# chagmgang/distributed_reinforcement_learning

Hardware: AMD Instinct MI355X
Metric: learner env-frames/sec (whole node), IMPALA deep-conv 84x84x4 (higher is better)
Workload: dtype bf16; 1 GPU; model=impala deep-conv 84x84x4 + LSTM256 V-trace, global_batch=32, seq_len=20, parallelism=dp1, num_action=18

## Files before the change

distributed_reinforcement_learning_amd/ops/conv_op.py:

```python

from __future__ import annotations

import torch

from distributed_reinforcement_learning_amd import ops as _ops

_LAYER_CO = {0: 32, 1: 32, 2: 64, 3: 64}

_WGRAD_STREAM = None


def _side_enabled() -> bool:
    import os
    return os.environ.get("DRLA_WGRAD_SIDE") == "1"


def wgrad_stream() -> torch.cuda.Stream:
    global _WGRAD_STREAM
    if _WGRAD_STREAM is None:
        _WGRAD_STREAM = torch.cuda.Stream()
    return _WGRAD_STREAM


def join_wgrad_stream() -> None:
    if _WGRAD_STREAM is not None:
        torch.cuda.current_stream().wait_stream(_WGRAD_STREAM)


STASH_INPUTS = False


class _ConvLayer(torch.autograd.Function):
    @staticmethod
    def forward(ctx, x: torch.Tensor, w_flat: torch.Tensor,
                bias_f32: torch.Tensor, layer: int):
        ext = _ops.require_ext()
        stash = STASH_INPUTS and layer <= 1
        y, x_st = ext.conv_fwd(layer, x.contiguous(), w_flat.contiguous(),
                               bias_f32.contiguous(), stash)
        ctx.save_for_backward(x_st if stash else x, w_flat, y)
        ctx.layer = layer
        return y

    @staticmethod
    def backward(ctx, dy: torch.Tensor):
        x, w_flat, y = ctx.saved_tensors
        ext = _ops.require_ext()
        layer = ctx.layer
        co = _LAYER_CO[layer]
        if not (dy.is_contiguous() or (dy.stride(-1) == 1
                                        and dy.dim() >= 2)):
            dy = dy.contiguous()
        dy_m = ext.relu_mask_bwd(dy, y, co, layer)
        if _side_enabled():
            cur = torch.cuda.current_stream()
            side = wgrad_stream()
            side.wait_stream(cur)
            with torch.cuda.stream(side):
                dw, dbias = ext.conv_wgrad(layer, x, dy_m)
            if not torch.cuda.is_current_stream_capturing():
                cur.wait_stream(side)
                for t in (dw, dbias):
                    t.record_stream(cur)
                for t in (x, dy_m):
                    t.record_stream(side)
        else:
            dw, dbias = ext.conv_wgrad(layer, x, dy_m)
        dx = None
        if layer >= 2 and ctx.needs_input_grad[0]:
            dx = ext.conv_dgrad(layer, dy_m, w_flat)
        return dx, dw, dbias, None


def conv_layer(x: torch.Tensor, conv: torch.nn.Conv2d,
               layer: int) -> torch.Tensor:
    w = conv.weight
    co = w.shape[0]
    w_flat = w.permute(0, 2, 3, 1).reshape(co, -1)
    return _ConvLayer.apply(x, w_flat, conv.bias, layer)


def atari_conv_stack(stack, x_u8_nhwc: torch.Tensor) -> torch.Tensor:
    ci = x_u8_nhwc.shape[-1]
    l1 = 0 if ci == 4 else 1
    y = conv_layer(x_u8_nhwc, stack.conv1, l1)
    y = conv_layer(y, stack.conv2, 2)
    y = conv_layer(y, stack.conv3, 3)
    return y.reshape(y.shape[0], -1)


def custom_stack_ok(stack, x: torch.Tensor) -> bool:
    return (x.is_cuda and x.dtype == torch.uint8
            and x.shape[1] == 84 and x.shape[2] == 84
            and x.shape[3] in (1, 4)
            and stack.conv1.weight.dtype == torch.bfloat16
            and _ops.available())
```

distributed_reinforcement_learning_amd/ops/hip/bind.cpp:

```cpp

#include <torch/extension.h>
#include <ATen/hip/HIPContext.h>
#include <hip/hip_runtime.h>

#include <algorithm>
#include <array>
#include <tuple>

#include "drla_kernels.h"

namespace {

hipStream_t cur_stream() {
  return at::hip::getCurrentHIPStream().stream();
}

void check_gpu_contig(const torch::Tensor& t, const char* name) {
  TORCH_CHECK(t.is_cuda(), name, " must be on the GPU");
  TORCH_CHECK(t.is_contiguous(), name, " must be contiguous");
}

template <typename... Ts>
void check_all_gpu_contig(const char* what, const Ts&... ts) {
  (check_gpu_contig(ts, what), ...);
// ... 133 lines not shown
                       0, cur_stream(), BF16P(in), BF16P(w), BF16P(bias),
                       BF16PM(out), batch);
  }
  return {out, x_stash};
}

static torch::Tensor& dbias_slot_buf(const torch::Tensor& like,
                                     int64_t slot_id) {
  static torch::Tensor bufs[4];
  TORCH_CHECK(slot_id >= 0 && slot_id < 4, "bad slot id");
  if (!bufs[slot_id].defined()) {
    bufs[slot_id] =
        torch::zeros({DRLA_DBIAS_SLOTS * DRLA_DBIAS_STRIDE},
                     like.options().dtype(torch::kFloat));
  }
  return bufs[slot_id];
}

torch::Tensor relu_mask_bwd(torch::Tensor dy, torch::Tensor y, int64_t CO,
                            int64_t slot_id) {
  check_gpu_contig(y, "y");
  TORCH_CHECK(dy.is_cuda(), "dy must be on GPU");
  long long n_stride, row_elems;
  if (dy.is_contiguous()) {
    n_stride = row_elems = dy.numel() / dy.size(0);
  } else {
    row_elems = 1;
    for (int d = 1; d < dy.dim(); ++d) {
      TORCH_CHECK(dy.stride(d - 1) >= dy.stride(d), "dy must be row-major");
      row_elems *= dy.size(d);
    }
    TORCH_CHECK(dy.stride(dy.dim() - 1) == 1 &&
                    dy.stride(0) >= row_elems && row_elems % 8 == 0,
                "dy view must be inner-contiguous");
    for (int d = 1; d + 1 < dy.dim(); ++d) {
      TORCH_CHECK(dy.stride(d) == dy.size(d + 1) * dy.stride(d + 1),
                  "dy inner dims must be contiguous");
    }
    n_stride = dy.stride(0);
  }
  auto out = torch::empty(dy.sizes(), dy.options());
  auto& slots = dbias_slot_buf(dy, slot_id);
  const long long n = dy.numel();
  TORCH_CHECK(n % 8 == 0, "relu_mask_bwd wants numel % 8 == 0");
  int grid = drla_grid(n / 8);
  if (grid > 640) grid = 640;
  hipLaunchKernelGGL(drla_relu_mask_bwd, dim3(grid), dim3(DRLA_BLOCK),
                     0, cur_stream(), BF16P(dy), BF16P(y), BF16PM(out),
                     slots.data_ptr<float>(), n, (int)CO, n_stride,
                     row_elems);
  return out;
}

std::tuple<torch::Tensor, torch::Tensor> conv_wgrad(int layer,
                                                    torch::Tensor in,
                                                    torch::Tensor dy) {
  check_gpu_contig(in, "in");
  check_gpu_contig(dy, "dy");
  const auto& cfg = conv_layer(layer);
  const int batch = in.size(0);
  const int K = cfg.kh * cfg.kw * cfg.ci;
  static int split_env = [] {
    const char* e = getenv("DRLA_WGRAD_SPLIT");
    return e ? atoi(e) : 0;
  }();
  const int split = split_env ? split_env : ((layer <= 1) ? 512 : 64);
  static torch::Tensor scratch_cache[4];
  if (!scratch_cache[layer].defined()) {
    scratch_cache[layer] =
        torch::zeros({K, cfg.co}, dy.options().dtype(torch::kFloat));
  }
  auto scratch = scratch_cache[layer];
  const dim3 grid((K + DRLA_CONV_WGRAD_BK - 1) / DRLA_CONV_WGRAD_BK, split);
  if (layer <= 1) {
    hipLaunchKernelGGL(kConvWgradU8[layer], grid, dim3(DRLA_CONV_BLOCK), 0,
                       cur_stream(), in.data_ptr<uint8_t>(), BF16P(dy),
                       scratch.data_ptr<float>(), batch);
  } else {
    hipLaunchKernelGGL(kConvWgradBf16[layer - 2], grid,
                       dim3(DRLA_CONV_BLOCK), 0, cur_stream(), BF16P(in),
                       BF16P(dy), scratch.data_ptr<float>(), batch);
  }
  auto dw = torch::empty({cfg.co, K}, dy.options().dtype(torch::kBFloat16));
  auto dbias = torch::empty({cfg.co}, dy.options().dtype(torch::kBFloat16));
  auto& slots = dbias_slot_buf(dy, layer);
  hipLaunchKernelGGL(drla_wgrad_finalize,
                     dim3(drla_grid((long long)K * cfg.co)),
                     dim3(DRLA_BLOCK), 0, cur_stream(),
                     scratch.data_ptr<float>(), BF16PM(dw), K, cfg.co,
                     slots.data_ptr<float>(), BF16PM(dbias));
  return {dw, dbias};
}

torch::Tensor conv_dgrad(int layer, torch::Tensor dy, torch::Tensor w) {
  check_gpu_contig(dy, "dy");
  check_gpu_contig(w, "w");
  TORCH_CHECK(layer == 2 || layer == 3, "dgrad only for l2/l3");
  const auto& cfg = conv_layer(layer);
  const int batch = dy.size(0);
  auto dx = torch::empty({batch, cfg.hi, cfg.wi, cfg.ci},
                         dy.options().dtype(torch::kBFloat16));
  if (layer == 2) {
    const int grid_c = conv_m_tiles(batch * (cfg.hi / 2) * (cfg.wi / 2));
    hipLaunchKernelGGL(drla_conv_dgrad_l2, dim3(grid_c, 4),
                       dim3(DRLA_CONV_BLOCK), 0, cur_stream(), BF16P(dy),
                       BF16P(w), BF16PM(dx), batch);
  } else {
    hipLaunchKernelGGL(drla_conv_dgrad_l3,
                       dim3(conv_m_tiles(batch * cfg.hi * cfg.wi)),
                       dim3(DRLA_CONV_BLOCK), 0, cur_stream(), BF16P(dy),
                       BF16P(w), BF16PM(dx), batch);
  }
  return dx;
}

std::tuple<torch::Tensor, torch::Tensor> dqn_loss_fwd(
    torch::Tensor main_q, torch::Tensor next_main, torch::Tensor next_tgt,
    torch::Tensor actions, torch::Tensor rewards, torch::Tensor discounts,
    torch::Tensor weights) {
  check_all_gpu_contig("dqn_loss input", main_q, next_main, next_tgt,
                       actions, rewards, discounts, weights);
  TORCH_CHECK(actions.scalar_type() == torch::kInt, "actions must be i32");
  const int B = main_q.size(0), A = main_q.size(1);
  const DualPtr mq = dual_ptr(main_q);
  auto fopt = rewards.options().dtype(torch::kFloat);
  auto loss = torch::zeros({1}, fopt);
  auto td = torch::empty({B}, fopt);
  hipLaunchKernelGGL(
      drla_dqn_loss_fwd, dim3((B + 255) / 256), dim3(256), 0, cur_stream(),
      mq.bf16, mq.f32, next_main.data_ptr<float>(), next_tgt.data_ptr<float>(),
      actions.data_ptr<int>(), rewards.data_ptr<float>(),
      discounts.data_ptr<float>(), weights.data_ptr<float>(),
      loss.data_ptr<float>(), td.data_ptr<float>(), B, A);
  return {loss, td};
}

torch::Tensor dqn_loss_bwd(torch::Tensor td, torch::Tensor actions,
                           torch::Tensor weights, torch::Tensor gloss,
                           int64_t A, bool want_bf16) {
  check_all_gpu_contig("dqn_loss bwd input", td, actions, weights, gloss);
  const int B = td.numel();
  auto dmq = torch::empty(
      {B, A},
      td.options().dtype(want_bf16 ? torch::kBFloat16 : torch::kFloat));
  const DualPtr out = dual_ptr(dmq);
  hipLaunchKernelGGL(
      drla_dqn_loss_bwd, dim3(((long long)B * A + 255) / 256), dim3(256), 0,
      cur_stream(), td.data_ptr<float>(), actions.data_ptr<int>(),
      weights.data_ptr<float>(), gloss.data_ptr<float>(), out.bf16, out.f32,
      B, (int)A);
  return dmq;
}

std::tuple<torch::Tensor, torch::Tensor, torch::Tensor> a2c_loss_fwd(
    torch::Tensor logits, torch::Tensor value, torch::Tensor next_value,
    torch::Tensor actions, torch::Tensor rewards, torch::Tensor done,
    double gamma, int64_t clip_mode, double c_bl, double c_ent) {
  check_all_gpu_contig("a2c loss input", logits, value, next_value, actions,
                       rewards, done);
  TORCH_CHECK(actions.scalar_type() == torch::kInt, "actions must be i32");
  TORCH_CHECK(done.scalar_type() == torch::kBool, "done must be bool");
  const int N = logits.size(0), A = logits.size(1);
  const DualPtr lg = dual_ptr(logits);
  auto fopt = value.options().dtype(torch::kFloat);
// ... 757 lines not shown
                     norm_buf.data_ptr<float>(), static_cast<float>(clip),
                     lr_buf.data_ptr<float>(), static_cast<float>(rho),
                     static_cast<float>(eps), n);
}

void rmsprop_step(torch::Tensor p, torch::Tensor g, torch::Tensor ms,
                  double clip, double lr, double rho, double eps) {
  auto lr_buf = torch::full({1}, lr, p.options());
  rmsprop_step_t(p, g, ms, clip, lr_buf, rho, eps);
}

void adam_step_t(torch::Tensor p, torch::Tensor g, torch::Tensor m,
                 torch::Tensor v, double clip, torch::Tensor lr_buf,
                 double beta1, double beta2, double eps) {
  check_all_gpu_contig("adam tensor", p, g, m, v, lr_buf);
  const long long n = p.numel();
  torch::Tensor norm_buf;
  if (clip > 0) {
    norm_buf = sq_norm(g);
  } else {
    norm_buf = torch::zeros({1}, p.options());
  }
  hipLaunchKernelGGL(drla_adam_step, dim3(drla_grid(n)), dim3(DRLA_BLOCK), 0,
                     cur_stream(), p.data_ptr<float>(), g.data_ptr<float>(),
                     m.data_ptr<float>(), v.data_ptr<float>(),
                     norm_buf.data_ptr<float>(), static_cast<float>(clip),
                     lr_buf.data_ptr<float>(), static_cast<float>(beta1),
                     static_cast<float>(beta2), static_cast<float>(eps), n);
}

void adam_step(torch::Tensor p, torch::Tensor g, torch::Tensor m,
               torch::Tensor v, double clip, double lr_t, double beta1,
               double beta2, double eps) {
  auto lr_buf = torch::full({1}, lr_t, p.options());
  adam_step_t(p, g, m, v, clip, lr_buf, beta1, beta2, eps);
}

}

PYBIND11_MODULE(TORCH_EXTENSION_NAME, m) {
  m.def("normalize_frames_f32", &normalize_frames_f32,
        "uint8 frames -> float32/255 (K11)");
  m.def("normalize_frames_bf16", &normalize_frames_bf16,
        "uint8 frames -> bf16/255 (K11)");
  m.def("vtrace_scan", &vtrace_scan, "fused V-trace reverse scan (K5)");
  m.def("vtrace_loss_fwd", &vtrace_loss_fwd,
        "fused IMPALA loss pipeline forward (K5+K7+K13)");
  m.def("vtrace_loss_bwd", &vtrace_loss_bwd,
        "fused IMPALA loss pipeline backward (closed form)");
  m.def("mfma_probe", &mfma_probe, "16x16x32 bf16 MFMA layout probe");
  m.def("conv_fwd", &conv_fwd,
        "MFMA implicit-GEMM conv fwd, fused normalize+bias+ReLU (K1)");
  m.def("conv_wgrad", &conv_wgrad, "MFMA conv weight gradient (K1 bwd)");
  m.def("conv_dgrad", &conv_dgrad, "MFMA conv data gradient (K1 bwd)");
  m.def("relu_mask_bwd", &relu_mask_bwd,
        "fused-ReLU backward mask + bias gradient");
  m.def("dqn_loss_fwd", &dqn_loss_fwd,
        "fused double-DQN target + IS-weighted TD loss (K8)");
  m.def("dqn_loss_bwd", &dqn_loss_bwd, "closed-form K8 backward");
  m.def("a2c_loss_fwd", &a2c_loss_fwd, "fused A2C loss fwd (K6)");
  m.def("a2c_loss_bwd", &a2c_loss_bwd, "fused A2C loss bwd (K6)");
  m.def("r2d2_loss_fwd", &r2d2_loss_fwd,
        "fused R2D2 sequence-TD tail fwd (K9; n_step > 1 or "
        "priority_eta >= 0 selects the n-step kernel)",
        py::arg("mq"), py::arg("tq"), py::arg("actions"), py::arg("rewards"),
        py::arg("done"), py::arg("weights"), py::arg("gamma"),
        py::arg("clip_mode"), py::arg("n_step") = 1,
        py::arg("priority_eta") = -1.0);
  m.def("dhead_train_fwd", &dhead_train_fwd,
        "grad-carrying dueling head fwd (R2D2 trained window)");
  m.def("dhead_train_bwd", &dhead_train_bwd,
        "grad-carrying dueling head bwd chain + weight grads");
  m.def("dueling_head_fwd", &dueling_head_fwd,
        "no-grad dueling head over the post-burn-in window");
  m.def("r2d2_loss_bwd", &r2d2_loss_bwd,
        "fused R2D2 sequence-TD tail bwd (K9)");
  m.def("per_update", &per_update, "GPU PER segment-tree batched update");
  m.def("per_sample", &per_sample, "GPU PER stratified sample descent");
  m.def("multi_gather", &multi_gather,
        "one-kernel replay batch gather (all fields)");
  m.def("per_rebuild", &per_rebuild,
        "GPU PER interior-sum rebuild (float32 drift repair)");
  m.def("embed_bwd", &embed_bwd,
        "action-embedding table gradient (K2 backward)");
  m.def("lstm_tail_fwd", &lstm_tail_fwd, "fused LSTM gate tail fwd (K3)");
  m.def("lstm_tail_bwd", &lstm_tail_bwd, "fused LSTM gate tail bwd (K3)");
  m.def("mlp_heads_fwd", &mlp_heads_fwd,
        "fused policy+value MLP heads forward (K4)");
  m.def("mlp_heads_bwd", &mlp_heads_bwd,
        "fused heads dgrad chain + ReLU masks + bias grads (K4 bwd)");
  m.def("embed_mlp_fwd", &embed_mlp_fwd,
        "fused action-embedding MLP forward (K2)");
  m.def("embed_mlp_bwd", &embed_mlp_bwd,
        "fused action-embedding MLP backward (K2 bwd)");
  m.def("mlp_heads_pack_wt", &mlp_heads_pack_wt,
        "one-kernel transposed-weight pack for the heads dgrad");
  m.def("mlp_heads_wgrad", &mlp_heads_wgrad,
        "all six head wgrads (dW = dz^T @ act) in one MFMA launch");
  m.def("lstm_seq_train_fwd", &lstm_seq_train_fwd,
        "grad-carrying whole-sequence LSTM forward (K3 seq, R2D2 train)");
  m.def("lstm_seq_train_bwd", &lstm_seq_train_bwd,
        "whole-sequence LSTM backward (one kernel over the recurrence)");
  m.def("lstm_seq_fwd", &lstm_seq_fwd,
        "whole no-grad LSTM unroll in one kernel (K3 seq / burn-in)");
  m.def("sq_norm", &sq_norm, "squared L2 norm of a flat tensor (K12)");
  m.def("grad_gather", &grad_gather,
        "one-kernel scattered-grad -> flat bucket pack (K12b)");
// ... 15 lines not shown
```

distributed_reinforcement_learning_amd/ops/hip/conv.hip:

```cpp

#include "drla_kernels.h"

#define CONV_KERNEL \
  extern "C" __global__ __launch_bounds__(DRLA_CONV_BLOCK) void

__device__ __forceinline__ float cv_bf2f(bf16raw u) {
  unsigned int x = ((unsigned int)u) << 16;
  return __uint_as_float(x);
}

extern "C" __global__ void drla_mfma_probe(const bf16raw* __restrict__ A,
                                           const bf16raw* __restrict__ B,
                                           float* __restrict__ D) {
  const int l = threadIdx.x;
  bf16x8 a_frag, b_frag;
  for (int e = 0; e < 8; ++e) {
    a_frag[e] = (short)A[(l & 15) * 32 + ((l >> 4) * 8 + e)];
    b_frag[e] = (short)B[((l >> 4) * 8 + e) * 16 + (l & 15)];
  }
  f32x4 acc = {0.f, 0.f, 0.f, 0.f};
  acc = __builtin_amdgcn_mfma_f32_16x16x32_bf16(a_frag, b_frag, acc, 0, 0, 0);
  for (int r = 0; r < 4; ++r) {
    D[((l >> 4) * 4 + r) * 16 + (l & 15)] = acc[r];
  }
// ... 242 lines not shown
    long long si = i;
    if (strided) {
      const long long r = i / row8;
      si = (r * n_stride + (i - r * row8) * 8) / 8;
    }
    const uint4 dv = dy4[si];
    const uint4 yv = y4[i];
    uint4 ov;
    DRLA_RM_LANE(dv.x, yv.x, ov.x, acc[0], acc[1]);
    DRLA_RM_LANE(dv.y, yv.y, ov.y, acc[2], acc[3]);
    DRLA_RM_LANE(dv.z, yv.z, ov.z, acc[4], acc[5]);
    DRLA_RM_LANE(dv.w, yv.w, ov.w, acc[6], acc[7]);
    out4[i] = ov;
  }
#undef DRLA_RM_LANE
  __shared__ float red[DRLA_BLOCK * 8];
  for (int e = 0; e < 8; ++e) red[tid * 8 + e] = acc[e];
  __syncthreads();
  if (tid < CO) {
    const int g = tid / 8;
    const int e = tid % 8;
    float s = 0.0f;
    for (int t = g; t < DRLA_BLOCK; t += CO / 8) s += red[t * 8 + e];
    atomicAdd(&dbias_slots[(blockIdx.x & (DRLA_DBIAS_SLOTS - 1)) *
                               DRLA_DBIAS_STRIDE +
                           tid], s);
  }
}

extern "C" __global__ void drla_wgrad_finalize(
    float* __restrict__ scratch, bf16raw* __restrict__ dw, int K,
    int CO, float* __restrict__ dbias_slots,
    bf16raw* __restrict__ dbias) {
  if (dbias_slots && blockIdx.x == 0 && (int)threadIdx.x < CO) {
    float s = 0.0f;
    for (int t = 0; t < DRLA_DBIAS_SLOTS; ++t) {
      s += dbias_slots[t * DRLA_DBIAS_STRIDE + threadIdx.x];
      dbias_slots[t * DRLA_DBIAS_STRIDE + threadIdx.x] = 0.0f;
    }
    dbias[threadIdx.x] = drla_f32_to_bf16(s);
  }
  long long i = blockIdx.x * (long long)blockDim.x + threadIdx.x;
  const long long total = (long long)K * CO;
  const long long stride = gridDim.x * (long long)blockDim.x;
  for (; i < total; i += stride) {
    const int co = i / K;
    const int k = i - (long long)co * K;
    const long long si = (long long)k * CO + co;
    dw[i] = drla_f32_to_bf16(scratch[si]);
    scratch[si] = 0.0f;
  }
}


template <typename IN_T, int CI, int CO, int KH, int KW, int STRIDE, int HI,
          int WI, int HO, int WO>
__device__ void conv_wgrad_impl(const IN_T* __restrict__ in,
                                const bf16raw* __restrict__ dy,
                                float* __restrict__ scratch,
                                int batch) {
  constexpr int K = KH * KW * CI;
  constexpr int BKM = 64;
  constexpr int BKK = DRLA_CONV_WGRAD_BK;
  constexpr int PAD = 8;
  constexpr int NFRAG = CO / 16;
  constexpr int CO_PER_T = (CO * 32) / DRLA_CONV_BLOCK;
  const int M = batch * HO * WO;

  __shared__ bf16raw Am[2][BKK][BKM + PAD];
  __shared__ bf16raw BmT[2][CO][BKM + PAD];

  const int tid = threadIdx.x;
  const int wave = tid / 64;
  const int lane = tid % 64;
  const int k_row0 = blockIdx.x * BKK;

  f32x4 acc[NFRAG];
  for (int ni = 0; ni < NFRAG; ++ni) acc[ni] = {0.f, 0.f, 0.f, 0.f};

  const int m_per_split = (M + gridDim.y - 1) / gridDim.y;
  const int m_begin = blockIdx.y * m_per_split;
  const int m_end = min(M, m_begin + m_per_split);

  const int a_m = tid >> 2;
  const int a_k = (tid & 3) * 16;
  long long a_off0 = 0, a_off1 = 0;
  long long a_offc[16];
  if constexpr (CI == 4) {
    const int kb = k_row0 + a_k;
    const int kh = kb / (KW * CI);
    a_off0 = (long long)kh * WI + (kb - kh * KW * CI) / CI;
  } else if constexpr (CI == 1) {
    static_assert(K % BKK == 0,
                  "CI==1 contiguous row staging requires K % BKK == 0");
#pragma unroll
    for (int t = 0; t < 16; ++t) {
      const int k2 = k_row0 + a_k + t;
      const int kh = k2 / KW;
      a_offc[t] = (k2 < K) ? (long long)kh * WI + (k2 - kh * KW) : -1;
    }
  } else {
    const int kk0 = k_row0 + a_k;
    const int kh0 = kk0 / (KW * CI);
    const int kwci0 = kk0 - kh0 * KW * CI;
    a_off0 = (kk0 < K)
        ? ((long long)kh0 * WI + kwci0 / CI) * CI + (kwci0 % CI) : -1;
// ... 144 lines not shown
  load_chunk(m_begin);
  store_chunk(0);
  load_chunk(m_begin + BKM);
  __syncthreads();
  int nchunks = 0;
  for (int m0 = m_begin; m0 < m_end; m0 += BKM) ++nchunks;
  for (int t = 0; t < nchunks; ++t) {
    const int cur = t & 1;
    if (t + 1 < nchunks) {
      store_chunk(1 - cur);
      load_chunk(m_begin + (long long)(t + 2) * BKM);
    }
    for (int kk = 0; kk < BKM; kk += 32) {
      const bf16x8 a_frag = *reinterpret_cast<const bf16x8*>(
          &Am[cur][wave * 16 + (lane & 15)][kk + (lane >> 4) * 8]);
      for (int ni = 0; ni < NFRAG; ++ni) {
        const int co = ni * 16 + (lane & 15);
        const bf16x8 b_frag = *reinterpret_cast<const bf16x8*>(
            &BmT[cur][co][kk + (lane >> 4) * 8]);
        acc[ni] = __builtin_amdgcn_mfma_f32_16x16x32_bf16(a_frag, b_frag,
                                                          acc[ni], 0, 0, 0);
      }
    }
    __syncthreads();
  }

  for (int ni = 0; ni < NFRAG; ++ni) {
    const int co = ni * 16 + (lane & 15);
    for (int r = 0; r < 4; ++r) {
      const int k = k_row0 + wave * 16 + (lane >> 4) * 4 + r;
      if (k < K) atomicAdd(&scratch[(long long)k * CO + co], acc[ni][r]);
    }
  }
}

CONV_KERNEL drla_conv_wgrad_l1(
    const unsigned char* in, const bf16raw* dy, float* scratch, int batch) {
  conv_wgrad_impl<unsigned char, DRLA_CONV_GEOM(0)>(in, dy, scratch, batch);
}
CONV_KERNEL drla_conv_wgrad_l1_c1(
    const unsigned char* in, const bf16raw* dy, float* scratch, int batch) {
  conv_wgrad_impl<unsigned char, DRLA_CONV_GEOM(1)>(in, dy, scratch, batch);
}
CONV_KERNEL drla_conv_wgrad_l2(
    const bf16raw* in, const bf16raw* dy, float* scratch, int batch) {
  conv_wgrad_impl<bf16raw, DRLA_CONV_GEOM(2)>(in, dy, scratch, batch);
}
CONV_KERNEL drla_conv_wgrad_l3(
    const bf16raw* in, const bf16raw* dy, float* scratch, int batch) {
  conv_wgrad_impl<bf16raw, DRLA_CONV_GEOM(3)>(in, dy, scratch, batch);
}


template <int CI, int CO, int KH, int KW, int STRIDE, int HI, int WI, int HO,
          int WO>
__device__ void conv_dgrad_impl(const bf16raw* __restrict__ dy,
                                const bf16raw* __restrict__ w,
                                bf16raw* __restrict__ dx,
                                int batch) {
  constexpr int K = KH * KW * CI;
  constexpr int Kg = KH * KW * CO;
  constexpr int BM = DRLA_CONV_BM;
  constexpr int BK = 32;
  constexpr int PAD = 8;
  constexpr int NFRAG = CI / 16;
  const int M2 = batch * HI * WI;

  __shared__ bf16raw Ad[BM][BK + PAD];
  __shared__ bf16raw Bd[CI][BK + PAD];

  const int tid = threadIdx.x;
  const int wave = tid / 64;
  const int lane = tid % 64;
  const int row0 = blockIdx.x * BM;

  f32x4 acc[2][NFRAG];
  for (int mi = 0; mi < 2; ++mi)
    for (int ni = 0; ni < NFRAG; ++ni)
      acc[mi][ni] = {0.f, 0.f, 0.f, 0.f};

  const int a_row = tid >> 1;
  const int a_k0 = (tid & 1) * 16;
  const int m2 = row0 + a_row;
  const int n_idx = m2 / (HI * WI);
  const int rem = m2 - n_idx * (HI * WI);
  const int hi = rem / WI;
  const int wi = rem - hi * WI;

  uint4 rda0, rda1;
  bf16raw rbw[8];
  constexpr int CI_PER_T = (CI * BK) / DRLA_CONV_BLOCK;
  const int b_col = tid % BK;
  const int b_ci0 = (tid / BK) * CI_PER_T;

  auto load_chunk = [&](int kg0) {
    const int tap = kg0 / CO;
    const int co0 = kg0 - tap * CO;
    const int kh = tap / KW;
    const int kw = tap - kh * KW;
    bool valid = (m2 < M2);
    int ho = 0, wo = 0;
    if (valid) {
      const int hh = hi - kh;
      const int ww = wi - kw;
      valid = hh >= 0 && ww >= 0 && (hh % STRIDE) == 0 && (ww % STRIDE) == 0;
      if (valid) {
        ho = hh / STRIDE;
        wo = ww / STRIDE;
        valid = ho < HO && wo < WO;
      }
    }
    if (valid) {
      const bf16raw* src =
          dy + ((long long)(n_idx * HO + ho) * WO + wo) * CO + co0 + a_k0;
      rda0 = *reinterpret_cast<const uint4*>(src);
      rda1 = *reinterpret_cast<const uint4*>(src + 8);
    } else {
      rda0 = uint4{0, 0, 0, 0};
      rda1 = uint4{0, 0, 0, 0};
    }
    const bf16raw* src = w + (long long)(co0 + b_col) * K + tap * CI + b_ci0;
#pragma unroll
    for (int e = 0; e < CI_PER_T; ++e) rbw[e] = src[e];
  };

  auto store_chunk = [&]() {
    *reinterpret_cast<uint4*>(&Ad[a_row][a_k0]) = rda0;
    *reinterpret_cast<uint4*>(&Ad[a_row][a_k0 + 8]) = rda1;
#pragma unroll
    for (int e = 0; e < CI_PER_T; ++e) Bd[b_ci0 + e][b_col] = rbw[e];
  };

  load_chunk(0);
  for (int kg0 = 0; kg0 < Kg; kg0 += BK) {
    store_chunk();
    __syncthreads();
    if (kg0 + BK < Kg) load_chunk(kg0 + BK);

    for (int mi = 0; mi < 2; ++mi) {
      const bf16x8 a_frag = *reinterpret_cast<const bf16x8*>(
          &Ad[wave * 32 + mi * 16 + (lane & 15)][(lane >> 4) * 8]);
      for (int ni = 0; ni < NFRAG; ++ni) {
        const bf16x8 b_frag = *reinterpret_cast<const bf16x8*>(
            &Bd[ni * 16 + (lane & 15)][(lane >> 4) * 8]);
        acc[mi][ni] = __builtin_amdgcn_mfma_f32_16x16x32_bf16(
            a_frag, b_frag, acc[mi][ni], 0, 0, 0);
      }
    }
    __syncthreads();
  }

  for (int mi = 0; mi < 2; ++mi) {
    for (int ni = 0; ni < NFRAG; ++ni) {
      const int ci = ni * 16 + (lane & 15);
      for (int r = 0; r < 4; ++r) {
        const int grow = row0 + wave * 32 + mi * 16 + (lane >> 4) * 4 + r;
        if (grow < M2) {
          dx[(long long)grow * CI + ci] = drla_f32_to_bf16(acc[mi][ni][r]);
        }
      }
    }
  }
}

template <int CI, int CO, int KH, int KW, int HI, int WI, int HO, int WO>
__device__ void conv_dgrad_s2_impl(const bf16raw* __restrict__ dy,
                                   const bf16raw* __restrict__ w,
                                   bf16raw* __restrict__ dx, int batch) {
  constexpr int K = KH * KW * CI;
  constexpr int BM = DRLA_CONV_BM;
  constexpr int BK = 32;
  constexpr int PAD = 8;
  constexpr int NFRAG = CI / 16;
  constexpr int H2 = HI / 2, W2 = WI / 2;
  const int ph = blockIdx.y >> 1, pw = blockIdx.y & 1;
  const int Mc = batch * H2 * W2;

  __shared__ bf16raw Ad[BM][BK + PAD];
  __shared__ bf16raw Bd[CI][BK + PAD];

  const int tid = threadIdx.x;
  const int wave = tid / 64;
  const int lane = tid % 64;
  const int row0 = blockIdx.x * BM;

  f32x4 acc[2][NFRAG];
  for (int mi = 0; mi < 2; ++mi)
    for (int ni = 0; ni < NFRAG; ++ni)
      acc[mi][ni] = {0.f, 0.f, 0.f, 0.f};

  const int a_row = tid >> 1;
  const int a_k0 = (tid & 1) * 16;
  const int mc = row0 + a_row;
  const int n_idx = mc / (H2 * W2);
  const int rem = mc - n_idx * (H2 * W2);
  const int hi = (rem / W2) * 2 + ph;
  const int wi = (rem - (rem / W2) * W2) * 2 + pw;

  uint4 rda0, rda1;
  bf16raw rbw[8];
  constexpr int CI_PER_T = (CI * BK) / DRLA_CONV_BLOCK;
  const int b_col = tid % BK;
  const int b_ci0 = (tid / BK) * CI_PER_T;
  constexpr int NIT = 4 * (CO / BK);

  auto load_chunk = [&](int it) {
    const int t = it / (CO / BK);
    const int co0 = (it - t * (CO / BK)) * BK;
    const int kh = ph + 2 * (t >> 1);
    const int kw = pw + 2 * (t & 1);
    bool valid = (mc < Mc);
    int ho = 0, wo = 0;
    if (valid) {
      const int hh = hi - kh;
      const int ww = wi - kw;
      valid = hh >= 0 && ww >= 0;
      if (valid) {
        ho = hh >> 1;
        wo = ww >> 1;
        valid = ho < HO && wo < WO;
      }
    }
    if (valid) {
      const bf16raw* src =
          dy + ((long long)(n_idx * HO + ho) * WO + wo) * CO + co0 + a_k0;
      rda0 = *reinterpret_cast<const uint4*>(src);
      rda1 = *reinterpret_cast<const uint4*>(src + 8);
    } else {
      rda0 = uint4{0, 0, 0, 0};
      rda1 = uint4{0, 0, 0, 0};
    }
    const int tap = kh * KW + kw;
    const bf16raw* src = w + (long long)(co0 + b_col) * K + tap * CI + b_ci0;
#pragma unroll
    for (int e = 0; e < CI_PER_T; ++e) rbw[e] = src[e];
  };

  auto store_chunk = [&]() {
    *reinterpret_cast<uint4*>(&Ad[a_row][a_k0]) = rda0;
    *reinterpret_cast<uint4*>(&Ad[a_row][a_k0 + 8]) = rda1;
#pragma unroll
    for (int e = 0; e < CI_PER_T; ++e) Bd[b_ci0 + e][b_col] = rbw[e];
  };

  load_chunk(0);
  for (int it = 0; it < NIT; ++it) {
    store_chunk();
    __syncthreads();
    if (it + 1 < NIT) load_chunk(it + 1);
    for (int mi = 0; mi < 2; ++mi) {
      const bf16x8 a_frag = *reinterpret_cast<const bf16x8*>(
          &Ad[wave * 32 + mi * 16 + (lane & 15)][(lane >> 4) * 8]);
      for (int ni = 0; ni < NFRAG; ++ni) {
        const bf16x8 b_frag = *reinterpret_cast<const bf16x8*>(
            &Bd[ni * 16 + (lane & 15)][(lane >> 4) * 8]);
        acc[mi][ni] = __builtin_amdgcn_mfma_f32_16x16x32_bf16(
            a_frag, b_frag, acc[mi][ni], 0, 0, 0);
      }
    }
    __syncthreads();
  }

  for (int mi = 0; mi < 2; ++mi) {
    for (int ni = 0; ni < NFRAG; ++ni) {
      const int ci = ni * 16 + (lane & 15);
      for (int r = 0; r < 4; ++r) {
        const int growc = row0 + wave * 32 + mi * 16 + (lane >> 4) * 4 + r;
        if (growc < Mc) {
          const int gn = growc / (H2 * W2);
          const int grem = growc - gn * (H2 * W2);
          const int ghi = (grem / W2) * 2 + ph;
          const int gwi = (grem - (grem / W2) * W2) * 2 + pw;
          dx[(((long long)gn * HI + ghi) * WI + gwi) * CI + ci] =
              drla_f32_to_bf16(acc[mi][ni][r]);
        }
      }
    }
  }
}

CONV_KERNEL drla_conv_dgrad_l2(
    const bf16raw* dy, const bf16raw* w, bf16raw* dx, int batch) {
  constexpr DrlaConvLayer g = DRLA_CONV_LAYERS[2];
  static_assert(g.stride == 2, "the parity-class dgrad is stride-2 only");
  conv_dgrad_s2_impl<g.ci, g.co, g.kh, g.kw, g.hi, g.wi, g.ho, g.wo>(
      dy, w, dx, batch);
}
CONV_KERNEL drla_conv_dgrad_l3(
    const bf16raw* dy, const bf16raw* w, bf16raw* dx, int batch) {
  conv_dgrad_impl<DRLA_CONV_GEOM(3)>(dy, w, dx, batch);
}
```

distributed_reinforcement_learning_amd/ops/hip/drla_common.h:

```cpp
#pragma once

#include <hip/hip_runtime.h>
#include <hip/hip_bf16.h>

typedef unsigned short bf16raw;
typedef __attribute__((ext_vector_type(4))) float f32x4;
typedef __attribute__((ext_vector_type(8))) short bf16x8;
typedef __attribute__((ext_vector_type(4))) unsigned short ushort4v;

#define DRLA_WAVE 64
#define DRLA_NORM_SLOTS 16
#define DRLA_DBIAS_SLOTS 16
#define DRLA_DBIAS_STRIDE 64
#define DRLA_BLOCK 256


struct DrlaConvLayer { int ci, co, kh, kw, stride, hi, wi, ho, wo; };
constexpr DrlaConvLayer DRLA_CONV_LAYERS[4] = {
    {4, 32, 8, 8, 4, 84, 84, 20, 20},
    {1, 32, 8, 8, 4, 84, 84, 20, 20},
    {32, 64, 4, 4, 2, 20, 20, 9, 9},
    {64, 64, 3, 3, 1, 9, 9, 7, 7},
};
#define DRLA_CONV_GEOM(l)                                               \
  DRLA_CONV_LAYERS[l].ci, DRLA_CONV_LAYERS[l].co, DRLA_CONV_LAYERS[l].kh, \
      DRLA_CONV_LAYERS[l].kw, DRLA_CONV_LAYERS[l].stride,               \
      DRLA_CONV_LAYERS[l].hi, DRLA_CONV_LAYERS[l].wi,                   \
      DRLA_CONV_LAYERS[l].ho, DRLA_CONV_LAYERS[l].wo
#define DRLA_CONV_BLOCK 256
#define DRLA_CONV_BM 128
#define DRLA_CONV_WGRAD_BK 64

#define VT_MAX_T 128
#define VT_MAX_A 64

#define MH_HID 256
#define MH_BM 16
#define MH_MAX_A 32

#define DHEAD_MAX_IN 256
#define DHEAD_MAX_MID 512
#define DHEAD_MAX_AO 64
#define DRLA_LDS_BUDGET (160 * 1024)
constexpr size_t drla_dhead_fwd_lds_bytes(int IN, int MID, int AO) {
  return (size_t)(MID * IN + AO * MID) * sizeof(bf16raw) +
         (size_t)(2 * MID + 2 * IN + 2 * AO) * sizeof(float);
}

#define LSTM_SEQ_MAX_GATES 1024
#define LSTM_SEQ_STATIC_LDS_BYTES (LSTM_SEQ_MAX_GATES * (int)sizeof(float))
constexpr int drla_lstm_seq_wh_elems(int H) { return H * 4 * H; }
constexpr int drla_lstm_seq_lds_bytes(int H, bool wh_in_lds = true) {
  return (wh_in_lds ? drla_lstm_seq_wh_elems(H) * (int)sizeof(bf16raw) : 0) +
         2 * H * (int)sizeof(float) + 16;
}
constexpr bool drla_lstm_seq_wh_fits_lds(int H) {
  return drla_lstm_seq_lds_bytes(H) + LSTM_SEQ_STATIC_LDS_BYTES <=
         DRLA_LDS_BUDGET;
}

#define DRLA_MAX_BLOCKS 2048

static inline int drla_grid(long long work_items, int block = DRLA_BLOCK) {
  long long blocks = (work_items + block - 1) / block;
  if (blocks > DRLA_MAX_BLOCKS) blocks = DRLA_MAX_BLOCKS;
  if (blocks < 1) blocks = 1;
  return static_cast<int>(blocks);
}

__device__ __forceinline__ int drla_clamp_idx(int a, int n) {
  return a < 0 ? 0 : (a >= n ? n - 1 : a);
}

__device__ __forceinline__ float drla_sigmoid(float x) {
  return 1.0f / (1.0f + __expf(-x));
}

__device__ __forceinline__ unsigned short drla_f32_to_bf16(float f) {
  __hip_bfloat162 v = __float22bfloat162_rn(float2{f, f});
  return *reinterpret_cast<unsigned short*>(&v);
}

__device__ __forceinline__ unsigned int drla_f32x2_to_bf16x2(float a,
                                                             float b) {
// ... 4 lines not shown
```

distributed_reinforcement_learning_amd/ops/hip/drla_kernels.h:

```cpp
#pragma once

#include <hip/hip_runtime.h>

#include "drla_common.h"

#define DRLA_KERNEL extern "C" __global__ void

DRLA_KERNEL drla_u8_normalize_f32(const uchar4*, float4*, long long);
DRLA_KERNEL drla_u8_normalize_bf16(const uchar4*, ushort4v*, long long);
DRLA_KERNEL drla_u8_normalize_f32_tail(const unsigned char*, float*,
                                       long long, long long);
DRLA_KERNEL drla_u8_normalize_bf16_tail(const unsigned char*, bf16raw*,
                                        long long, long long);
DRLA_KERNEL drla_embed_bwd_scatter(const long long*, const bf16raw*,
                                   const float*, float*, long long, int,
                                   long long);
DRLA_KERNEL drla_f32_to_bf16_zero_kernel(float*, bf16raw*, long long);

DRLA_KERNEL drla_vtrace_scan(const float*, const float*, const float*,
                             float*, int, int);

DRLA_KERNEL drla_vtrace_loss_fwd(
    const bf16raw*, const float*, const float*, const float*, const int*,
    const float*, const unsigned char*, float, int, float, float, float*,
// ... 15 lines not shown
                                    float*, long long, int, long long);
DRLA_KERNEL drla_lstm_seq_fwd(
    const bf16raw*, const float*, const bf16raw*, const float*, const float*,
    const unsigned char*, float*, float*, float*, float, int, int, int);
DRLA_KERNEL drla_lstm_seq_fwd_gmem(
    const bf16raw*, const float*, const bf16raw*, const float*, const float*,
    const unsigned char*, float*, float*, float*, float, int, int, int);
DRLA_KERNEL drla_lstm_seq_train_fwd(
    const bf16raw*, const bf16raw*, const float*, const float*,
    const unsigned char*, float*, float*, float*, float*, float*, bf16raw*,
    float, int, int, int);
DRLA_KERNEL drla_lstm_seq_train_bwd(
    const float*, const float*, const float*, const float*, const float*,
    const bf16raw*, const unsigned char*, bf16raw*, float*, float*, int, int,
    int);

DRLA_KERNEL drla_sq_norm(const float*, float*, long long);
DRLA_KERNEL drla_sq_norm_bf16(const bf16raw*, float*, long long);
DRLA_KERNEL drla_rmsprop_step(float*, const float*, float*, const float*,
                              float, const float*, float, float, long long);
DRLA_KERNEL drla_rmsprop_step_bf16(bf16raw*, const bf16raw*, float*, float*,
                                   const float*, float, const float*, float,
                                   float, long long);
DRLA_KERNEL drla_adam_step(float*, const float*, float*, float*,
                           const float*, float, const float*, float, float,
                           float, long long);
DRLA_KERNEL drla_adam_step_bf16(bf16raw*, const bf16raw*, float*, float*,
                                float*, const float*, float, const float*,
                                float, float, float, long long);
DRLA_KERNEL drla_grad_gather(const unsigned long long*, const long long*,
                             const long long*, bf16raw*, int, long long,
                             float*, int);

DRLA_KERNEL drla_mfma_probe(const bf16raw*, const bf16raw*, float*);
DRLA_KERNEL drla_conv_fwd_l1(const unsigned char*, const bf16raw*,
                             const bf16raw*, bf16raw*, int, unsigned char*);
DRLA_KERNEL drla_conv_fwd_l1_c1(const unsigned char*, const bf16raw*,
                                const bf16raw*, bf16raw*, int,
                                unsigned char*);
DRLA_KERNEL drla_conv_fwd_l2(const bf16raw*, const bf16raw*, const bf16raw*,
                             bf16raw*, int);
DRLA_KERNEL drla_conv_fwd_l3(const bf16raw*, const bf16raw*, const bf16raw*,
                             bf16raw*, int);
DRLA_KERNEL drla_relu_mask_bwd(const bf16raw*, const bf16raw*, bf16raw*,
                               float*, long long, int, long long, long long);
DRLA_KERNEL drla_wgrad_finalize(float*, bf16raw*, int, int, float*,
                                bf16raw*);
DRLA_KERNEL drla_conv_wgrad_l1(const unsigned char*, const bf16raw*, float*,
                               int);
DRLA_KERNEL drla_conv_wgrad_l1_c1(const unsigned char*, const bf16raw*,
                                  float*, int);
DRLA_KERNEL drla_conv_wgrad_l2(const bf16raw*, const bf16raw*, float*, int);
DRLA_KERNEL drla_conv_wgrad_l3(const bf16raw*, const bf16raw*, float*, int);
DRLA_KERNEL drla_conv_dgrad_l2(const bf16raw*, const bf16raw*, bf16raw*,
                               int);
DRLA_KERNEL drla_conv_dgrad_l3(const bf16raw*, const bf16raw*, bf16raw*,
                               int);

DRLA_KERNEL drla_per_update(float*, const long long*, const float*, int,
                            long long);
DRLA_KERNEL drla_per_rebuild_level(float*, long long, long long);
DRLA_KERNEL drla_multi_gather(const long long*, const unsigned long long*,
                              const unsigned long long*, const long long*,
                              int);
DRLA_KERNEL drla_per_sample(const float*, const float*, const float*,
                            long long*, float*, int, long long);

DRLA_KERNEL drla_dqn_loss_fwd(
    const bf16raw*, const float*, const float*, const float*, const int*,
    const float*, const float*, const float*, float*, float*, int, int);
DRLA_KERNEL drla_dqn_loss_bwd(const float*, const int*, const float*,
                              const float*, bf16raw*, float*, int, int);

DRLA_KERNEL drla_a2c_loss_fwd(
    const bf16raw*, const float*, const float*, const float*, const int*,
    const float*, const unsigned char*, float, int, float, float, float*,
    float*, float*, int, int);
DRLA_KERNEL drla_a2c_loss_bwd(const float*, const float*, const int*,
                              const float*, int, float, float, bf16raw*,
                              float*, float*, int, int);

DRLA_KERNEL drla_r2d2_loss_fwd(
    const bf16raw*, const float*, const bf16raw*, const float*, const int*,
    const float*, const unsigned char*, const float*, float, int, float*,
    float*, float*, int, int, int);
DRLA_KERNEL drla_r2d2_nstep_loss_fwd(
    const bf16raw*, const float*, const bf16raw*, const float*, const int*,
    const float*, const unsigned char*, const float*, float, int, int, float,
    float*, float*, float*, int, int, int);
DRLA_KERNEL drla_r2d2_loss_bwd(const float*, const int*, const float*,
                               const float*, bf16raw*, float*, int, int,
                               int);
DRLA_KERNEL drla_dueling_head_fwd(
    const float*, const bf16raw*, const bf16raw*, const bf16raw*,
    const bf16raw*, bf16raw*, int, int, int, int, int, int);
DRLA_KERNEL drla_dhead_train_fwd(
    const float*, const bf16raw*, const bf16raw*, const bf16raw*,
    const bf16raw*, bf16raw*, bf16raw*, int, int, int, int);
DRLA_KERNEL drla_dhead_train_bwd(
    const bf16raw*, const bf16raw*, const float*, const bf16raw*,
    const bf16raw*, float*, float*, int, int, int, int);
DRLA_KERNEL drla_dhead_train_fin(const float*, bf16raw*, bf16raw*, bf16raw*,
                                 bf16raw*, int, int, int);

DRLA_KERNEL drla_mlp_heads_fwd(
    const float*, const bf16raw*, const bf16raw*, const bf16raw*,
    const bf16raw*, const bf16raw*, const bf16raw*, const bf16raw*,
    const bf16raw*, const bf16raw*, const bf16raw*, const bf16raw*,
    const bf16raw*, bf16raw*, float*, bf16raw*, int, int);
DRLA_KERNEL drla_mlp_heads_bwd(
// ... 25 lines not shown
```

Baseline: 999,000 frames/s.

## Fuse conv stack backward: dgrad with ReLU mask, batched wgrad finalize

```diff
diff --git a/distributed_reinforcement_learning_amd/ops/conv_op.py b/distributed_reinforcement_learning_amd/ops/conv_op.py
--- a/distributed_reinforcement_learning_amd/ops/conv_op.py
+++ b/distributed_reinforcement_learning_amd/ops/conv_op.py
@@ -72,6 +72,43 @@
         return dx, dw, dbias, None
 
 
+def _unfused() -> bool:
+    import os
+    return os.environ.get("DRLA_CONV_UNFUSED") == "1" or _side_enabled()
+
+
+class _ConvStack(torch.autograd.Function):
+
+    @staticmethod
+    def forward(ctx, x, w1, b1, w2, b2, w3, b3, l1: int):
+        ext = _ops.require_ext()
+        stash = STASH_INPUTS
+        w2, w3 = w2.contiguous(), w3.contiguous()
+        y1, x_st = ext.conv_fwd(l1, x.contiguous(), w1.contiguous(),
+                                b1.contiguous(), stash)
+        y2, _ = ext.conv_fwd(2, y1, w2, b2.contiguous(), False)
+        y3, _ = ext.conv_fwd(3, y2, w3, b3.contiguous(), False)
+        y3 = y3.view(y3.shape[0], -1)
+        ctx.save_for_backward(x_st if stash else x, y1, y2, y3, w2, w3)
+        ctx.l1 = l1
+        return y3
+
+    @staticmethod
+    def backward(ctx, dy3: torch.Tensor):
+        x, y1, y2, y3, w2, w3 = ctx.saved_tensors
+        ext = _ops.require_ext()
+        l1 = ctx.l1
+        if not (dy3.is_contiguous() or (dy3.stride(-1) == 1
+                                         and dy3.dim() >= 2)):
+            dy3 = dy3.contiguous()
+        dy_m3 = ext.relu_mask_bwd(dy3, y3, 64, 3).view(-1, 7, 7, 64)
+        dy_m2 = ext.conv_dgrad(3, dy_m3, w3, y_below=y2, below_slot=2)
+        dy_m1 = ext.conv_dgrad(2, dy_m2, w2, y_below=y1, below_slot=l1)
+        (dw3, db3), (dw2, db2), (dw1, db1) = ext.conv_wgrad(
+            [3, 2, l1], [y2, y1, x], [dy_m3, dy_m2, dy_m1])
+        return None, dw1, db1, dw2, db2, dw3, db3, None
+
+
 def conv_layer(x: torch.Tensor, conv: torch.nn.Conv2d,
                layer: int) -> torch.Tensor:
     w = conv.weight
@@ -83,6 +120,12 @@
 def atari_conv_stack(stack, x_u8_nhwc: torch.Tensor) -> torch.Tensor:
     ci = x_u8_nhwc.shape[-1]
     l1 = 0 if ci == 4 else 1
+    if not _unfused():
+        flat = []
+        for conv in (stack.conv1, stack.conv2, stack.conv3):
+            w = conv.weight
+            flat += [w.permute(0, 2, 3, 1).reshape(w.shape[0], -1), conv.bias]
+        return _ConvStack.apply(x_u8_nhwc, *flat, l1)
     y = conv_layer(x_u8_nhwc, stack.conv1, l1)
     y = conv_layer(y, stack.conv2, 2)
     y = conv_layer(y, stack.conv3, 3)
diff --git a/distributed_reinforcement_learning_amd/ops/hip/bind.cpp b/distributed_reinforcement_learning_amd/ops/hip/bind.cpp
--- a/distributed_reinforcement_learning_amd/ops/hip/bind.cpp
+++ b/distributed_reinforcement_learning_amd/ops/hip/bind.cpp
@@ -209,9 +209,8 @@
   return out;
 }
 
-std::tuple<torch::Tensor, torch::Tensor> conv_wgrad(int layer,
-                                                    torch::Tensor in,
-                                                    torch::Tensor dy) {
+torch::Tensor conv_wgrad_accumulate(int layer, const torch::Tensor& in,
+                                    const torch::Tensor& dy) {
   check_gpu_contig(in, "in");
   check_gpu_contig(dy, "dy");
   const auto& cfg = conv_layer(layer);
@@ -238,6 +237,15 @@
                        dim3(DRLA_CONV_BLOCK), 0, cur_stream(), BF16P(in),
                        BF16P(dy), scratch.data_ptr<float>(), batch);
   }
+  return scratch;
+}
+
+std::tuple<torch::Tensor, torch::Tensor> conv_wgrad(int layer,
+                                                    torch::Tensor in,
+                                                    torch::Tensor dy) {
+  auto scratch = conv_wgrad_accumulate(layer, in, dy);
+  const auto& cfg = conv_layer(layer);
+  const int K = cfg.kh * cfg.kw * cfg.ci;
   auto dw = torch::empty({cfg.co, K}, dy.options().dtype(torch::kBFloat16));
   auto dbias = torch::empty({cfg.co}, dy.options().dtype(torch::kBFloat16));
   auto& slots = dbias_slot_buf(dy, layer);
@@ -249,7 +257,46 @@
   return {dw, dbias};
 }
 
-torch::Tensor conv_dgrad(int layer, torch::Tensor dy, torch::Tensor w) {
+std::vector<std::tuple<torch::Tensor, torch::Tensor>> conv_wgrad_stack(
+    std::vector<int64_t> layers, std::vector<torch::Tensor> ins,
+    std::vector<torch::Tensor> dys) {
+  const size_t n = layers.size();
+  TORCH_CHECK(n >= 1 && n <= DRLA_FINALIZE_MAX_LAYERS,
+              "conv_wgrad takes 1..", DRLA_FINALIZE_MAX_LAYERS, " layers");
+  TORCH_CHECK(ins.size() == n && dys.size() == n,
+              "conv_wgrad: layers, ins and dys must have one length");
+  for (size_t j = 0; j < n; ++j) {
+    for (size_t i = 0; i < j; ++i) {
+      TORCH_CHECK(layers[i] != layers[j],
+                  "conv_wgrad: a layer's scratch holds one gradient at a time");
+    }
+  }
+  DrlaWgradFinalizeArgs args{};
+  args.n = (int)n;
+  std::vector<std::tuple<torch::Tensor, torch::Tensor>> out;
+  int blocks = 0;
+  for (size_t j = 0; j < n; ++j) {
+    const int layer = (int)layers[j];
+    auto scratch = conv_wgrad_accumulate(layer, ins[j], dys[j]);
+    const auto& cfg = conv_layer(layer);
+    const int K = cfg.kh * cfg.kw * cfg.ci;
+    const auto bf16 = dys[j].options().dtype(torch::kBFloat16);
+    auto dw = torch::empty({cfg.co, K}, bf16);
+    auto dbias = torch::empty({cfg.co}, bf16);
+    args.layer[j] = {scratch.data_ptr<float>(), BF16PM(dw),
+                     dbias_slot_buf(dys[j], layer).data_ptr<float>(),
+                     BF16PM(dbias), K, cfg.co, blocks};
+    blocks += (K * cfg.co + DRLA_BLOCK - 1) / DRLA_BLOCK;
+    out.emplace_back(dw, dbias);
+  }
+  hipLaunchKernelGGL(drla_wgrad_finalize_multi, dim3(blocks),
+                     dim3(DRLA_BLOCK), 0, cur_stream(), args);
+  return out;
+}
+
+torch::Tensor conv_dgrad(int layer, torch::Tensor dy, torch::Tensor w,
+                         c10::optional<torch::Tensor> y_below,
+                         int64_t below_slot) {
   check_gpu_contig(dy, "dy");
   check_gpu_contig(w, "w");
   TORCH_CHECK(layer == 2 || layer == 3, "dgrad only for l2/l3");
@@ -257,16 +304,28 @@
   const int batch = dy.size(0);
   auto dx = torch::empty({batch, cfg.hi, cfg.wi, cfg.ci},
                          dy.options().dtype(torch::kBFloat16));
+  const bf16raw* yp = nullptr;
+  float* slotp = nullptr;
+  if (y_below.has_value()) {
+    check_gpu_contig(*y_below, "y_below");
+    TORCH_CHECK(y_below->sizes() == dx.sizes(),
+                "y_below must have the dgrad output's shape");
+    TORCH_CHECK(layer == 3 ? below_slot == 2
+                           : (below_slot == 0 || below_slot == 1),
+                "below_slot must name the layer that produced y_below");
+    yp = BF16P(*y_below);
+    slotp = dbias_slot_buf(dy, below_slot).data_ptr<float>();
+  }
   if (layer == 2) {
     const int grid_c = conv_m_tiles(batch * (cfg.hi / 2) * (cfg.wi / 2));
     hipLaunchKernelGGL(drla_conv_dgrad_l2, dim3(grid_c, 4),
                        dim3(DRLA_CONV_BLOCK), 0, cur_stream(), BF16P(dy),
-                       BF16P(w), BF16PM(dx), batch);
+                       BF16P(w), BF16PM(dx), batch, yp, slotp);
   } else {
     hipLaunchKernelGGL(drla_conv_dgrad_l3,
                        dim3(conv_m_tiles(batch * cfg.hi * cfg.wi)),
                        dim3(DRLA_CONV_BLOCK), 0, cur_stream(), BF16P(dy),
-                       BF16P(w), BF16PM(dx), batch);
+                       BF16P(w), BF16PM(dx), batch, yp, slotp);
   }
   return dx;
 }
@@ -1130,7 +1189,14 @@
   m.def("conv_fwd", &conv_fwd,
         "MFMA implicit-GEMM conv fwd, fused normalize+bias+ReLU (K1)");
   m.def("conv_wgrad", &conv_wgrad, "MFMA conv weight gradient (K1 bwd)");
-  m.def("conv_dgrad", &conv_dgrad, "MFMA conv data gradient (K1 bwd)");
+  m.def("conv_wgrad", &conv_wgrad_stack,
+        "list form (layers, ins, dys): all wgrads, then one finalize; "
+        "returns [(dw, dbias), ...]");
+  m.def("conv_dgrad", &conv_dgrad,
+        "MFMA conv data gradient (K1 bwd); with y_below, fused with the "
+        "layer below's ReLU mask and bias-grad partials",
+        py::arg("layer"), py::arg("dy"), py::arg("w"),
+        py::arg("y_below") = py::none(), py::arg("below_slot") = -1);
   m.def("relu_mask_bwd", &relu_mask_bwd,
         "fused-ReLU backward mask + bias gradient");
   m.def("dqn_loss_fwd", &dqn_loss_fwd,
diff --git a/distributed_reinforcement_learning_amd/ops/hip/conv.hip b/distributed_reinforcement_learning_amd/ops/hip/conv.hip
--- a/distributed_reinforcement_learning_amd/ops/hip/conv.hip
+++ b/distributed_reinforcement_learning_amd/ops/hip/conv.hip
@@ -318,6 +318,34 @@
   }
 }
 
+extern "C" __global__ void drla_wgrad_finalize_multi(
+    DrlaWgradFinalizeArgs args) {
+  DrlaWgradFinalizeLayer L = args.layer[0];
+#pragma unroll
+  for (int j = 1; j < DRLA_FINALIZE_MAX_LAYERS; ++j) {
+    if (j < args.n && (int)blockIdx.x >= args.layer[j].block0) {
+      L = args.layer[j];
+    }
+  }
+  const int lb = blockIdx.x - L.block0;
+  if (lb == 0 && (int)threadIdx.x < L.CO) {
+    float s = 0.0f;
+    for (int t = 0; t < DRLA_DBIAS_SLOTS; ++t) {
+      s += L.dbias_slots[t * DRLA_DBIAS_STRIDE + threadIdx.x];
+      L.dbias_slots[t * DRLA_DBIAS_STRIDE + threadIdx.x] = 0.0f;
+    }
+    L.dbias[threadIdx.x] = drla_f32_to_bf16(s);
+  }
+  const int i = lb * (int)blockDim.x + threadIdx.x;
+  if (i < L.K * L.CO) {
+    const int co = i / L.K;
+    const int k = i - co * L.K;
+    const int si = k * L.CO + co;
+    L.dw[i] = drla_f32_to_bf16(L.scratch[si]);
+    L.scratch[si] = 0.0f;
+  }
+}
+
 
 template <typename IN_T, int CI, int CO, int KH, int KW, int STRIDE, int HI,
           int WI, int HO, int WO>
@@ -568,12 +596,75 @@
 }
 
 
+template <int CI, int NFRAG, typename RowOff>
+__device__ __forceinline__ unsigned int dgrad_y_load(
+    const bf16raw* __restrict__ y_below, int lane, RowOff row_off,
+    bf16raw (&yraw)[2 * NFRAG * 4]) {
+  static_assert(2 * NFRAG * 4 <= 32, "mask bits must fit one register");
+  unsigned int valid = 0;
+  long long offs[8];
+#pragma unroll
+  for (int mi = 0; mi < 2; ++mi) {
+#pragma unroll
+    for (int r = 0; r < 4; ++r) offs[mi * 4 + r] = row_off(mi, r);
+  }
+#pragma unroll
+  for (int mi = 0; mi < 2; ++mi) {
+#pragma unroll
+    for (int r = 0; r < 4; ++r) {
+      const long long off = offs[mi * 4 + r];
+      const bf16raw* src = y_below + (off >= 0 ? off : 0) + (lane & 15);
+#pragma unroll
+      for (int ni = 0; ni < NFRAG; ++ni) {
+        const int b = (mi * NFRAG + ni) * 4 + r;
+        yraw[b] = src[ni * 16];
+        if (off >= 0) valid |= 1u << b;
+      }
+    }
+  }
+  return valid;
+}
+
+template <int NFRAG>
+__device__ __forceinline__ unsigned int dgrad_y_mask(
+    const bf16raw (&yraw)[2 * NFRAG * 4], unsigned int valid) {
+  unsigned int mask = 0;
+#pragma unroll
+  for (int b = 0; b < 2 * NFRAG * 4; ++b) {
+    if (cv_bf2f(yraw[b]) > 0.0f) mask |= 1u << b;
+  }
+  return mask & valid;
+}
+
+template <int CI, int NFRAG>
+__device__ __forceinline__ void dgrad_bias_partials(
+    const float (&colsum)[NFRAG], float* red, float* __restrict__ below_slots,
+    int linear_block, int tid) {
+  const int wave = tid / 64;
+  const int lane = tid % 64;
+#pragma unroll
+  for (int ni = 0; ni < NFRAG; ++ni) {
+    red[(wave * 4 + (lane >> 4)) * CI + ni * 16 + (lane & 15)] = colsum[ni];
+  }
+  __syncthreads();
+  if (tid < CI) {
+    float s = 0.0f;
+#pragma unroll
+    for (int g = 0; g < 16; ++g) s += red[g * CI + tid];
+    atomicAdd(&below_slots[(linear_block & (DRLA_DBIAS_SLOTS - 1)) *
+                               DRLA_DBIAS_STRIDE +
+                           tid], s);
+  }
+}
+
 template <int CI, int CO, int KH, int KW, int STRIDE, int HI, int WI, int HO,
           int WO>
 __device__ void conv_dgrad_impl(const bf16raw* __restrict__ dy,
                                 const bf16raw* __restrict__ w,
                                 bf16raw* __restrict__ dx,
-                                int batch) {
+                                int batch,
+                                const bf16raw* __restrict__ y_below,
+                                float* __restrict__ below_slots) {
   constexpr int K = KH * KW * CI;
   constexpr int Kg = KH * KW * CO;
   constexpr int BM = DRLA_CONV_BM;
@@ -647,8 +738,7 @@
     for (int e = 0; e < CI_PER_T; ++e) Bd[b_ci0 + e][b_col] = rbw[e];
   };
 
-  load_chunk(0);
-  for (int kg0 = 0; kg0 < Kg; kg0 += BK) {
+  auto k_step = [&](int kg0) {
     store_chunk();
     __syncthreads();
     if (kg0 + BK < Kg) load_chunk(kg0 + BK);
@@ -664,25 +754,58 @@
       }
     }
     __syncthreads();
-  }
-
+  };
+
+  const bool masked = (y_below != nullptr);
+  unsigned int ymask = 0;
+  load_chunk(0);
+  if (masked) {
+    bf16raw yraw[2 * NFRAG * 4];
+    const unsigned int valid =
+        dgrad_y_load<CI, NFRAG>(y_below, lane, [&](int mi, int r) {
+          const int grow = row0 + wave * 32 + mi * 16 + (lane >> 4) * 4 + r;
+          return grow < M2 ? (long long)grow * CI : -1LL;
+        }, yraw);
+    k_step(0);
+    ymask = dgrad_y_mask<NFRAG>(yraw, valid);
+  } else {
+    k_step(0);
+  }
+  for (int kg0 = BK; kg0 < Kg; kg0 += BK) k_step(kg0);
+
+  float colsum[NFRAG];
+  for (int ni = 0; ni < NFRAG; ++ni) colsum[ni] = 0.0f;
   for (int mi = 0; mi < 2; ++mi) {
     for (int ni = 0; ni < NFRAG; ++ni) {
       const int ci = ni * 16 + (lane & 15);
       for (int r = 0; r < 4; ++r) {
         const int grow = row0 + wave * 32 + mi * 16 + (lane >> 4) * 4 + r;
+        bf16raw v = drla_f32_to_bf16(acc[mi][ni][r]);
+        if (masked) {
+          if (!((ymask >> ((mi * NFRAG + ni) * 4 + r)) & 1u)) v = 0;
+          colsum[ni] += cv_bf2f(v);
+        }
         if (grow < M2) {
-          dx[(long long)grow * CI + ci] = drla_f32_to_bf16(acc[mi][ni][r]);
-        }
-      }
-    }
+          dx[(long long)grow * CI + ci] = v;
+        }
+      }
+    }
+  }
+  if (masked) {
+    static_assert(sizeof(Ad) >= 16 * CI * sizeof(float),
+                  "column-sum staging must fit the A tile");
+    dgrad_bias_partials<CI, NFRAG>(colsum,
+                                   reinterpret_cast<float*>(&Ad[0][0]),
+                                   below_slots, blockIdx.x, tid);
   }
 }
 
 template <int CI, int CO, int KH, int KW, int HI, int WI, int HO, int WO>
 __device__ void conv_dgrad_s2_impl(const bf16raw* __restrict__ dy,
                                    const bf16raw* __restrict__ w,
-                                   bf16raw* __restrict__ dx, int batch) {
+                                   bf16raw* __restrict__ dx, int batch,
+                                   const bf16raw* __restrict__ y_below,
+                                   float* __restrict__ below_slots) {
   constexpr int K = KH * KW * CI;
   constexpr int BM = DRLA_CONV_BM;
   constexpr int BK = 32;
@@ -759,8 +882,18 @@
     for (int e = 0; e < CI_PER_T; ++e) Bd[b_ci0 + e][b_col] = rbw[e];
   };
 
-  load_chunk(0);
-  for (int it = 0; it < NIT; ++it) {
+  auto dx_row_off = [&](int growc) -> long long {
+    const bool in_range = growc < Mc;
+    const int g = in_range ? growc : 0;
+    const int gn = g / (H2 * W2);
+    const int grem = g - gn * (H2 * W2);
+    const int ghi = (grem / W2) * 2 + ph;
+    const int gwi = (grem - (grem / W2) * W2) * 2 + pw;
+    const long long off = (((long long)gn * HI + ghi) * WI + gwi) * CI;
+    return in_range ? off : -1LL;
+  };
+
+  auto k_step = [&](int it) {
     store_chunk();
     __syncthreads();
     if (it + 1 < NIT) load_chunk(it + 1);
@@ -775,34 +908,61 @@
       }
     }
     __syncthreads();
-  }
-
+  };
+
+  const bool masked = (y_below != nullptr);
+  unsigned int ymask = 0;
+  load_chunk(0);
+  if (masked) {
+    bf16raw yraw[2 * NFRAG * 4];
+    const unsigned int valid =
+        dgrad_y_load<CI, NFRAG>(y_below, lane, [&](int mi, int r) {
+          return dx_row_off(row0 + wave * 32 + mi * 16 + (lane >> 4) * 4 +
+                            r);
+        }, yraw);
+    k_step(0);
+    ymask = dgrad_y_mask<NFRAG>(yraw, valid);
+  } else {
+    k_step(0);
+  }
+  for (int it = 1; it < NIT; ++it) k_step(it);
+
+  float colsum[NFRAG];
+  for (int ni = 0; ni < NFRAG; ++ni) colsum[ni] = 0.0f;
   for (int mi = 0; mi < 2; ++mi) {
-    for (int ni = 0; ni < NFRAG; ++ni) {
-      const int ci = ni * 16 + (lane & 15);
-      for (int r = 0; r < 4; ++r) {
-        const int growc = row0 + wave * 32 + mi * 16 + (lane >> 4) * 4 + r;
-        if (growc < Mc) {
-          const int gn = growc / (H2 * W2);
-          const int grem = growc - gn * (H2 * W2);
-          const int ghi = (grem / W2) * 2 + ph;
-          const int gwi = (grem - (grem / W2) * W2) * 2 + pw;
-          dx[(((long long)gn * HI + ghi) * WI + gwi) * CI + ci] =
-              drla_f32_to_bf16(acc[mi][ni][r]);
-        }
-      }
-    }
+    for (int r = 0; r < 4; ++r) {
+      const long long off =
+          dx_row_off(row0 + wave * 32 + mi * 16 + (lane >> 4) * 4 + r);
+      for (int ni = 0; ni < NFRAG; ++ni) {
+        const int ci = ni * 16 + (lane & 15);
+        bf16raw v = drla_f32_to_bf16(acc[mi][ni][r]);
+        if (masked) {
+          if (!((ymask >> ((mi * NFRAG + ni) * 4 + r)) & 1u)) v = 0;
+          colsum[ni] += cv_bf2f(v);
+        }
+        if (off >= 0) dx[off + ci] = v;
+      }
+    }
+  }
+  if (masked) {
+    static_assert(sizeof(Ad) >= 16 * CI * sizeof(float),
+                  "column-sum staging must fit the A tile");
+    dgrad_bias_partials<CI, NFRAG>(
+        colsum, reinterpret_cast<float*>(&Ad[0][0]), below_slots,
+        blockIdx.y * gridDim.x + blockIdx.x, tid);
   }
 }
 
 CONV_KERNEL drla_conv_dgrad_l2(
-    const bf16raw* dy, const bf16raw* w, bf16raw* dx, int batch) {
+    const bf16raw* dy, const bf16raw* w, bf16raw* dx, int batch,
+    const bf16raw* y_below, float* below_slots) {
   constexpr DrlaConvLayer g = DRLA_CONV_LAYERS[2];
   static_assert(g.stride == 2, "the parity-class dgrad is stride-2 only");
   conv_dgrad_s2_impl<g.ci, g.co, g.kh, g.kw, g.hi, g.wi, g.ho, g.wo>(
-      dy, w, dx, batch);
+      dy, w, dx, batch, y_below, below_slots);
 }
 CONV_KERNEL drla_conv_dgrad_l3(
-    const bf16raw* dy, const bf16raw* w, bf16raw* dx, int batch) {
-  conv_dgrad_impl<DRLA_CONV_GEOM(3)>(dy, w, dx, batch);
-}
+    const bf16raw* dy, const bf16raw* w, bf16raw* dx, int batch,
+    const bf16raw* y_below, float* below_slots) {
+  conv_dgrad_impl<DRLA_CONV_GEOM(3)>(dy, w, dx, batch, y_below, below_slots);
+}
diff --git a/distributed_reinforcement_learning_amd/ops/hip/drla_common.h b/distributed_reinforcement_learning_amd/ops/hip/drla_common.h
--- a/distributed_reinforcement_learning_amd/ops/hip/drla_common.h
+++ b/distributed_reinforcement_learning_amd/ops/hip/drla_common.h
@@ -30,6 +30,19 @@
 #define DRLA_CONV_BLOCK 256
 #define DRLA_CONV_BM 128
 #define DRLA_CONV_WGRAD_BK 64
+
+#define DRLA_FINALIZE_MAX_LAYERS 3
+struct DrlaWgradFinalizeLayer {
+  float* scratch;
+  bf16raw* dw;
+  float* dbias_slots;
+  bf16raw* dbias;
+  int K, CO, block0;
+};
+struct DrlaWgradFinalizeArgs {
+  DrlaWgradFinalizeLayer layer[DRLA_FINALIZE_MAX_LAYERS];
+  int n;
+};
 
 #define VT_MAX_T 128
 #define VT_MAX_A 64
diff --git a/distributed_reinforcement_learning_amd/ops/hip/drla_kernels.h b/distributed_reinforcement_learning_amd/ops/hip/drla_kernels.h
--- a/distributed_reinforcement_learning_amd/ops/hip/drla_kernels.h
+++ b/distributed_reinforcement_learning_amd/ops/hip/drla_kernels.h
@@ -91,10 +91,11 @@
                                   float*, int);
 DRLA_KERNEL drla_conv_wgrad_l2(const bf16raw*, const bf16raw*, float*, int);
 DRLA_KERNEL drla_conv_wgrad_l3(const bf16raw*, const bf16raw*, float*, int);
+DRLA_KERNEL drla_wgrad_finalize_multi(DrlaWgradFinalizeArgs);
 DRLA_KERNEL drla_conv_dgrad_l2(const bf16raw*, const bf16raw*, bf16raw*,
-                               int);
+                               int, const bf16raw*, float*);
 DRLA_KERNEL drla_conv_dgrad_l3(const bf16raw*, const bf16raw*, bf16raw*,
-                               int);
+                               int, const bf16raw*, float*);
 
 DRLA_KERNEL drla_per_update(float*, const long long*, const float*, int,
                             long long);
```

After: 1.004 million frames/s (median of 2 runs). No clear change (+0.5%).
